# HJakeCunningham/ASVGP

Hardware: AMD Instinct MI355X
Metric: Mpoints/s per ELBO+grad step, N=10M 1D Matern-3/2 M=2048 (higher is better)
Workload: dtype f64

## Files before the change

### asvgp_amd/csrc/bcr_mfma.hpp

```cpp
#pragma once
#include "bcr.hpp"
#include "prior_plan.hpp"

namespace asvgp {

constexpr int BM_THREADS = 1024;
constexpr int BM_B = 4;
constexpr int BM_GAT = 0, BM_GBT = 16, BM_DINV = 32, BM_SD = 48, BM_CAT = 64, BM_CBT = 80, BM_W = 96, BM_DG = 100, BM_REC = 104;

__host__ __device__ inline size_t bcr_mfma_ws_doubles(long nb) { return (size_t)nb * BM_REC + 64; }
__host__ __device__ inline size_t bcr_mfma_lds_doubles(long nb) {
  return (size_t)((nb + 1) / 2 + 1) * 32 + (size_t)nb * 4 + 96 + (size_t)(BM_THREADS / 64) * 4 * 40 + (size_t)(nb / 8 + 2) * 52;
}

__device__ __forceinline__ double bm_mfma(double a, double b, double c) { return __builtin_amdgcn_mfma_f64_4x4x4f64(a, b, c, 0, 0, 0); }

__device__ __forceinline__ double bm_chol_linv(const double (&d)[10], int hi, int lo, double& dprod, int& badj) {
  double l00, i0, l10, l20, l30, l11, i1, l21, l31, l22, i2, l32, l33, i3;
  Num<double>::sqrt_inv(d[0], l00, i0);
  badj = !(d[0] > 0.0) ? 1 : 0;
  l10 = d[1] * i0; l20 = d[3] * i0; l30 = d[6] * i0;
  double s = fma(-l10, l10, d[2]);
  badj = (!(s > 0.0) && !badj) ? 2 : badj;
  Num<double>::sqrt_inv(s, l11, i1);
// ... 10 lines not shown
  const double z0 = (lo == 0) ? i0 : 0.0;
  const double z1 = fma(-l10, z0, (lo == 1) ? 1.0 : 0.0) * i1;
  const double z2 = fma(-l21, z1, fma(-l20, z0, (lo == 2) ? 1.0 : 0.0)) * i2;
  const double z3 = fma(-l32, z2, fma(-l31, z1, fma(-l30, z0, (lo == 3) ? 1.0 : 0.0))) * i3;
  return hi == 0 ? z0 : (hi == 1 ? z1 : (hi == 2 ? z2 : z3));
}

template <typename Src> __device__ __forceinline__ auto bm_src_load(const Src& A, int dd, long col, long M, int) -> decltype(A.load_dc(dd, col, M)) {
  return A.load_dc(dd, col, M);
}
template <typename Src> __device__ __forceinline__ double bm_src_load(const Src& A, int dd, long col, long M, long) {
  return A.load((long)dd * M + col, true);
}
struct BmLog {
  double m; int e;
  __device__ __forceinline__ void mul(double p) {
    m *= p;
    const int hi = __double2hiint(m);
    e += ((hi >> 20) & 0x7ff) - 1023;
    m = __hiloint2double((hi & 0x800fffff) | 0x3ff00000, __double2loint(m));
  }
};

__device__ __forceinline__ unsigned long long bm_wave_xor(unsigned long long x) {
#pragma unroll
  for (int off = 32; off > 0; off >>= 1) x ^= (unsigned long long)__shfl_xor((long long)x, off, 64);
  return x;
}
__device__ __forceinline__ void bm_msg_send(double* box, int n, double v, unsigned long long tag, int lane) {
  unsigned long long* b = reinterpret_cast<unsigned long long*>(box);
  const unsigned long long w = lane < n ? (unsigned long long)__double_as_longlong(v) : 0ull;
  const unsigned long long x = bm_wave_xor(w) ^ tag;
  if (lane < n) __hip_atomic_store(b + lane, w, __ATOMIC_RELAXED, __HIP_MEMORY_SCOPE_AGENT);
  if (lane == n) __hip_atomic_store(b + n, x, __ATOMIC_RELAXED, __HIP_MEMORY_SCOPE_AGENT);
}
__device__ __forceinline__ bool bm_msg_recv(const double* box, int n, double& v, unsigned long long tag, int lane, long spin_limit) {
  const unsigned long long* b = reinterpret_cast<const unsigned long long*>(box);
  for (long spins = 0; spins <= spin_limit; ++spins) {
    const unsigned long long w = lane <= n ? __hip_atomic_load(b + lane, __ATOMIC_RELAXED, __HIP_MEMORY_SCOPE_AGENT) : 0ull;
    const unsigned long long x = bm_wave_xor(lane < n ? w : 0ull) ^ tag;
    const unsigned long long chk = (unsigned long long)__shfl((long long)w, n, 64);
    if (x == chk) { v = __longlong_as_double((long long)w); return true; }
    __builtin_amdgcn_s_sleep(1);
  }
  return false;
}

struct BmSplit {
  int half = -1;
  double* xchg = nullptr;
  long spin_limit = 0;
  int* gave_up = nullptr;
  unsigned long long tag = 0;
};
constexpr int BM_XCHG = 96;

template <typename Src>
__device__ __attribute__((always_inline)) void bcr_mfma_solve(Src A, const double* rhs, int M, double* ws, double* lds, double* Sband, double* x,
                                                              double* logdet, int* info, int rhs_stride = 1, double* stamps = nullptr,
                                                              BmSplit sp = BmSplit{}) {
  constexpr int B = BM_B;
  const int tid = threadIdx.x;
  const int lane = tid & 63, wv = __builtin_amdgcn_readfirstlane(tid >> 6);
  const int r = lane >> 4, q = (lane >> 2) & 3, c = lane & 3;
  const int e = r * 4 + c, et = c * 4 + r;
  const int hi = r > c ? r : c, lo = r > c ? c : r;
  const int nb = (M + B - 1) / B;
  const int nslot = (nb + 1) / 2;
  double* Dl = lds;
  double* El = lds + (size_t)(nslot + 1) * 16;
  double* xs = El + (size_t)(nslot + 1) * 16;
  double* red = xs + (size_t)nb * B;
  double* slab = red + 96 + (size_t)(wv * 4 + q) * 40;
  double* Fl = red + 96 + (size_t)(BM_THREADS / 64) * 4 * 40;
  double* Sl = lds;
  int levels = 0;
  while ((1 << levels) < nb) ++levels;
  const bool split = sp.half >= 0;
  const int top = levels - 1, ht = 1 << (top > 0 ? top : 0);
  double s_other = 0.0;
  int bad_other = 0x7fffffff;
  auto level_share = [&](int l, int ne, int& m0, int& ne_h) {
    m0 = 0; ne_h = ne;
    if (!split) return;
    if (l < top) {
      const int mL = ht >> (l + 1);
      if (sp.half == 0) ne_h = ne < mL ? ne : mL;
      else { m0 = mL; ne_h = ne > mL ? ne - mL : 0; }
    } else {
      ne_h = sp.half == 0 ? ne : 0;
    }
  };
  int bad = 0;
  BmLog ld{1.0, 0};
  unsigned long long t_prev = stamps ? __builtin_amdgcn_s_memtime() : 0ull;
  int nst = 0;
  auto stamp = [&]() {
    if (stamps && tid == 0) { const unsigned long long t = __builtin_amdgcn_s_memtime(); stamps[nst++] = (double)(t - t_prev); t_prev = t; }
  };
  auto rec = [&](int node) -> double* { return ws + (size_t)node * BM_REC; };
  auto bandD = [&](int n, int rr, int cc) -> double {
    const int col = n * B + cc, row = n * B + rr;
    const bool pad = row >= M;
    const double v = bm_src_load(A, rr - cc, pad ? 0 : col, (long)M, 0);
    return pad ? ((rr == cc) ? 1.0 : 0.0) : v;
  };
// ... 264 lines not shown
        if (c == 0) xs[i * B + r] = w - gx;
        if (l >= 2) {
          double* Rw = Sl + (size_t)(i >> 2) * 48;
          Rw[e] = sii; Rw[16 + e] = -ncat; Rw[32 + e] = -ncbt;
        }
        if (l > 0) {
          double* Rw = rec(i);
          Rw[BM_SD + e] = sii; Rw[BM_CAT + e] = -ncat; Rw[BM_CBT + e] = -ncbt;
        }
        if (r >= c && i * B + r < M) Sband[(long)(r - c) * M + i * B + c] = sii;
        if (l == 0) {
          if (c <= r && i * B + c < M) Sband[(long)(B + c - r) * M + a * B + r] = -ncat;
          if (hasb && r <= c && b * B + r < M) Sband[(long)(B + r - c) * M + i * B + c] = -ncbt;
        }
      }
    }
    if (l == 1) __syncthreads(); else bcr_lds_barrier();
    if (split && l == top) {
      double* Rs = Sl + (size_t)(ht >> 2) * 48;
      if (sp.half == 0) {
        if (wv == 0) bm_msg_send(sp.xchg + 32, 52, lane < 48 ? Rs[lane < 48 ? lane : 0] : (lane < 52 ? xs[ht * B + lane - 48] : 0.0), sp.tag | 3ull, lane);
      } else {
        if (wv == 0) {
          double v = 0.0;
          if (!bm_msg_recv(sp.xchg + 32, 52, v, sp.tag | 3ull, lane, sp.spin_limit)) { if (lane == 0) *sp.gave_up = 1; }
          else if (lane < 48) {
            Rs[lane] = v;
            rec(ht)[BM_SD + lane] = v;
            if (lane < 16) {
              const int rr = lane >> 2, cc = lane & 3;
              if (rr >= cc && ht * B + rr < M) Sband[(long)(rr - cc) * M + ht * B + cc] = v;
            }
          } else if (lane < 52) {
            xs[ht * B + lane - 48] = v;
          }
        }
        __syncthreads();
        if (*sp.gave_up) return;
      }
    }
    stamp();
  }
  if (!(split && sp.half == 0))
    for (int col = M - B + tid; col < M; col += BM_THREADS)
      if (col >= 0)
#pragma unroll
        for (int dd = 1; dd <= B; ++dd)
          if (col + dd >= M) Sband[(long)dd * M + col] = 0.0;
  {
    const int row0 = (split && sp.half == 1) ? (ht + 1) * B : 0, row1 = (split && sp.half == 0) ? (ht + 1) * B : M;
    for (int row = row0 + tid; row < row1 && row < M; row += BM_THREADS) x[(long)row * rhs_stride] = xs[row];
  }
  if (!(split && sp.half == 1)) {
    const double mine = (r == 0 && c == 0) ? (log(ld.m) + (double)ld.e * 0.6931471805599453094) : 0.0;
    const double tot = wave_sum_dpp(mine);
    int bm = bad ? bad : 0x7fffffff;
#pragma unroll
    for (int off = 32; off > 0; off >>= 1) { const int o = __shfl_xor(bm, off, 64); bm = o < bm ? o : bm; }
    int* sbad = reinterpret_cast<int*>(red + 32);
    if (lane == 0) { red[wv] = tot; sbad[wv] = bm; }
    __syncthreads();
    if (split && tid == 0) { s_other = red[48]; bad_other = (int)red[49]; }
    if (tid == 0) {
      double s = 0.0;
      int bmin = 0x7fffffff;
      for (int w2 = 0; w2 < BM_THREADS / 64; ++w2) { s += red[w2]; bmin = sbad[w2] < bmin ? sbad[w2] : bmin; }
      s += s_other;
      bmin = bad_other < bmin ? bad_other : bmin;
      __hip_atomic_store(logdet + 0, 2.0 * s, __ATOMIC_RELAXED, __HIP_MEMORY_SCOPE_AGENT);
      __hip_atomic_store(logdet + 1, 0.0, __ATOMIC_RELAXED, __HIP_MEMORY_SCOPE_AGENT);
      __hip_atomic_store(info, (bmin == 0x7fffffff) ? 0 : bmin, __ATOMIC_RELAXED, __HIP_MEMORY_SCOPE_AGENT);
    }
  }
  stamp();
}


__host__ __device__ inline size_t bcr_mfma_pre_ws_doubles(long nb) { return (size_t)nb * 96 + 64; }
__host__ __device__ inline size_t bcr_mfma_pre_lds_doubles(long nb, int n_rec) {
  return PRIOR_TAB_HEADER + (size_t)2 * n_rec * prior_rec_fields(BM_B) + (size_t)(nb / 4 + 2) * 96 + (size_t)(nb + 1) / 2 + 64;
}

struct BmDual { double v, d; };
__device__ __forceinline__ BmDual bm_dmfma(BmDual x, BmDual y, BmDual c) {
  BmDual r;
  r.v = bm_mfma(x.v, y.v, c.v);
  r.d = bm_mfma(x.d, y.v, c.d);
  r.d = bm_mfma(x.v, y.d, r.d);
  return r;
}

__device__ __attribute__((always_inline)) void bcr_mfma_backward_pre(const double* __restrict__ tab, int n_rec, const int* __restrict__ node_rec, int M,
                                                                      double* ws, double* lds, double* Sv, double* Sd, double* logdet, int* info,
                                                                      unsigned long long* done_flag, unsigned long long seq,
                                                                      const unsigned long long* ready_flag = nullptr, long spin_limit = 0, int* gave_up = nullptr) {
  constexpr int B = BM_B, W = prior_rec_fields(B);
  const int tid = threadIdx.x;
  if (ready_flag) {
    if (tid == 0) {
      long spins = 0;
      while (__hip_atomic_load(ready_flag, __ATOMIC_RELAXED, __HIP_MEMORY_SCOPE_SYSTEM) < seq) {
        __builtin_amdgcn_s_sleep(8);
        if (++spins > spin_limit) { *gave_up = 1; break; }
      }
    }
    __syncthreads();
    if (*gave_up) return;
    __builtin_amdgcn_fence(__ATOMIC_ACQUIRE, "");
  }
// ... 107 lines not shown
```

### asvgp_amd/csrc/elbo.hip

```cpp
#include <stdlib.h>
#include <time.h>
#include <string.h>

#include "bcr_pre.hpp"
#include "bcr_mfma.hpp"
#include "handle.hpp"

namespace asvgp {


struct Ws {
  double *Kuu, *dK, *P, *LK, *dLK, *LP, *SK, *dSK, *SP, *c, *alpha, *logdets, *fin, *bcrK, *bcrP;
};
static size_t bcr_ws_chain(int planes, int k, bool big) {
  long ns = 1024;
  while ((long)planes * 2 * k * k * ns * 8 + 2 * ns * k * 8 + 1024 > 150 * 1024) ns >>= 1;
  if (big) ns *= 2;
  return (size_t)planes * (7 * k * k + k) * 2 * ns + (big ? (size_t)planes * k * k * ns : 0);
}
static size_t bcr_ws_K(int k, long M) {
  size_t a = bcr_ws_chain(2, k, false), b = bcr_ws_chain(2, k, true), c = bcr_pre_ws_doubles(k, (M + k - 1) / k);
  a = a > b ? a : b;
  return (a > c ? a : c) + 64;
}
// ... 348 lines not shown
    bcr_solve<double, K, 1, BandSumP, BIG>(BandSumP{A, Kuu, 1.0 / s}, b, M, wsP, lds, BandOut<double>{SP, nullptr}, x, logdets + 2, info + 1, nullptr, D);
    more_columns<K, BIG>(b, x, D, M, wsP, lds, lds_doubles);
  } else if (blockIdx.x == 1) {
    bcr_backward_pre<K>(tab, n_rec, node_rec, M, wsK, lds, BandOut<Dual>{SK, dSK}, logdets, info, done_flag, seq);
  } else {
    for (long e = (long)(blockIdx.x - 2) * blockDim.x + threadIdx.x; e < E; e += (long)fin.n_helpers * blockDim.x)
      assemble_band_slice(S_static, cf.c, cf.dc, cf.n, E, e, Kuu, dK);
    __syncthreads();
    if (threadIdx.x == 0) {
      __threadfence();
      __hip_atomic_fetch_add(fin.assembled, 1u, __ATOMIC_RELEASE, __HIP_MEMORY_SCOPE_AGENT);
    }
  }
  if (!fin.finalize) return;
  if (blockIdx.x < 2) {
    __syncthreads();
    if (threadIdx.x == 0) {
      __threadfence();
      __hip_atomic_fetch_add(fin.arrived, 1u, __ATOMIC_RELEASE, __HIP_MEMORY_SCOPE_AGENT);
    }
    return;
  }
  if (threadIdx.x == 0) {
    long spins = 0;
    while (__hip_atomic_load(fin.arrived, __ATOMIC_RELAXED, __HIP_MEMORY_SCOPE_AGENT) < 2u) {
      __builtin_amdgcn_s_sleep(8);
      if (++spins > (1L << 25)) { gave_up = 1; break; }
    }
  }
  __syncthreads();
  if (gave_up) { if (threadIdx.x == 0) atomicExch(info + 1, -1); return; }
  __builtin_amdgcn_fence(__ATOMIC_ACQUIRE, "agent");
  elbo_finalize_body<K>((int)blockIdx.x - 2, fin.n_helpers, lds, fin.stats, Kuu, dK, nullptr, nullptr, SK, dSK, SP, nullptr, x, logdets, (long)M, fin.D,
                        fin.th, fin.alpha_scale, fin.gacc, fin.ticket, fin.arrived, fin.out);
}

template <int K>
__global__ __launch_bounds__(BM_THREADS) void elbo_chains_mfma_kernel(KuuInterior ki, const double* S_static, KuuCoefs2 cf, double* Kuu, double* dK, const double* A, const double* b, int M,
                                                                      double* wsP, double* SP, double* x, double* logdets, int* info,
                                                                      double s, const double* tab, int n_rec, const int* node_rec,
                                                                      double* wsK, double* SK, double* dSK,
                                                                      unsigned long long* done_flag, unsigned long long seq,
                                                                      const unsigned long long* ready_flag, long spin_limit, FusedFin fin, const ThetaBox* box) {
  extern __shared__ double lds[];
  static_assert(K == BM_B, "matrix-core chains: bandwidth 4");
  const long E = (long)(K + 1) * M;
  const unsigned long long t_start = fin.debug_stamps ? __builtin_amdgcn_s_memrealtime() : 0ull;
  auto rstamp = [&](int slot) {
    if (fin.debug_stamps && threadIdx.x == 0 && blockIdx.x <= 2)
      logdets[(slot < 4 ? 8 + 4 * (int)blockIdx.x : 24) + slot] = (slot == 0) ? (double)(t_start & 0xffffffffull) : (double)((__builtin_amdgcn_s_memrealtime() - t_start) & 0xffffffffull);
  };
  rstamp(0);
  __shared__ int gave_up, kuu_ok;
  __shared__ double kuu_pref[4];
  if (threadIdx.x == 0) { gave_up = 0; kuu_ok = 0; }
  __syncthreads();
  double s_v = s, asc_v = fin.alpha_scale;
  ElboScalars th_v = fin.th;
  if (box) {
    if (threadIdx.x == 0) {
      long spins = 0;
      for (;;) {
        const unsigned long long got = __hip_atomic_load(&box->seq, __ATOMIC_RELAXED, __HIP_MEMORY_SCOPE_SYSTEM);
        if (got == seq) break;
        if (got == ~0ull || ++spins > spin_limit) { gave_up = 1; break; }
        __builtin_amdgcn_s_sleep(2);
      }
    }
    __syncthreads();
    if (gave_up) { if (threadIdx.x == 0) atomicExch(info + 1, -1); return; }
    s_v = box->s; asc_v = box->alpha_scale;
    th_v.v = box->v; th_v.l = box->l; th_v.s = box->s; th_v.N = box->N; th_v.Nw = box->Nw; th_v.cw = box->cw;
  }
  const double* stats = fin.stats;
  enum { LOGK, LOGP, TRKA, DTRKA, SKDK, SPDK, SKK, SPK, SPA, CC, AKA, ADKA, AAA, BA, NACC };
  double acc[NACC];
#pragma unroll
  for (int i = 0; i < NACC; ++i) acc[i] = 0.0;
  const bool isP = blockIdx.x == 0 || (fin.split && blockIdx.x == 2);
  const bool isPR = fin.split && blockIdx.x == 2;
  __shared__ double kdl[16];
  __shared__ double bnd[2 * PRIOR_BND_DIAGS * PRIOR_BND], dkb[2 * 5 * KI_DKB];
  {
    if (isP) rstamp(1);
    if (threadIdx.x == 0) {
      if (box) {
#pragma unroll
        for (int i = 0; i < 5; ++i) { kdl[i] = box->k[i]; kdl[8 + i] = box->dk[i]; }
      } else {
        kdl[0] = ki.k[0]; kdl[1] = ki.k[1]; kdl[2] = ki.k[2]; kdl[3] = ki.k[3]; kdl[4] = ki.k[4];
        kdl[8] = ki.dk[0]; kdl[9] = ki.dk[1]; kdl[10] = ki.dk[2]; kdl[11] = ki.dk[3]; kdl[12] = ki.dk[4];
      }
    }
    {
      const double* bnd_g = box ? box->bnd : reinterpret_cast<const double*>((const char*)__builtin_amdgcn_kernarg_segment_ptr() + offsetof(KuuInterior, bnd));
      const double* dkb_g = box ? box->dkb : reinterpret_cast<const double*>((const char*)__builtin_amdgcn_kernarg_segment_ptr() + offsetof(KuuInterior, dkb));
      if (threadIdx.x < 2 * PRIOR_BND_DIAGS * PRIOR_BND) bnd[threadIdx.x] = bnd_g[threadIdx.x];
      else if (threadIdx.x < 2 * PRIOR_BND_DIAGS * PRIOR_BND + 2 * 5 * KI_DKB) dkb[threadIdx.x - 2 * PRIOR_BND_DIAGS * PRIOR_BND] = dkb_g[threadIdx.x - 2 * PRIOR_BND_DIAGS * PRIOR_BND];
    }
    __syncthreads();
  }
  if (isP) {
    BmSplit bsp;
    if (fin.split) { bsp.half = isPR ? 1 : 0; bsp.xchg = fin.xchg; bsp.spin_limit = spin_limit; bsp.gave_up = &gave_up; bsp.tag = seq << 8; }
    bcr_mfma_solve<BandSumToep>(BandSumToep{A, 1.0 / s_v, (lds_cdouble_ptr)kdl, (lds_cdouble_ptr)bnd, ki.lo, ki.hi}, b, M, wsP, lds, SP, x, logdets + 2, info + 1, 1,
                                fin.debug_stamps ? (isPR ? fin.xchg + 128 : logdets + 32) : (double*)nullptr, bsp);
    rstamp(3);
    __syncthreads();
    if (gave_up) { if (threadIdx.x == 0) atomicExch(info + 1, -1); return; }
    rstamp(4);
    if (fin.finalize) {
      const double* xs_l = lds + (size_t)2 * ((((M + K - 1) / K) + 1) / 2 + 1) * 16;
      static_assert(BM_THREADS == 1024, "two columns per thread");
      int nbl = (M + K - 1) / K, lv = 0;
      while ((1 << lv) < nbl) ++lv;
      const long jsep = (long)(1 << (lv > 0 ? lv - 1 : 0)) * K;
      const long j0 = isPR ? jsep : 0, j1 = (fin.split && !isPR) ? jsep : (long)M;
      unsigned long long kw = 0ull;
      const bool kuu_reader = !isPR && (threadIdx.x >> 6) == 1;
      if (kuu_reader && (threadIdx.x & 63) <= 4)
        kw = __hip_atomic_load(reinterpret_cast<const unsigned long long*>(fin.gacc + 8) + (threadIdx.x & 63), __ATOMIC_RELAXED, __HIP_MEMORY_SCOPE_AGENT);
      double sp[2][K + 1], av[2][K + 1], bj[2];
#pragma unroll
      for (int cI = 0; cI < 2; ++cI) {
        const long j = j0 + threadIdx.x + cI * BM_THREADS, jc = j < j1 ? j : j1 - 1;
#pragma unroll
        for (int r = 0; r <= K; ++r) { sp[cI][r] = SP[(long)r * M + jc]; av[cI][r] = stats[(long)r * M + jc]; }
        bj[cI] = stats[(long)(K + 1) * M + jc];
      }
#pragma unroll
      for (int cI = 0; cI < 2; ++cI) {
        const long j = j0 + threadIdx.x + cI * BM_THREADS;
        if (j >= j1) continue;
        const bool left = j < ki.lo, right = j >= ki.hi;
        const double xj = xs_l[j];
#pragma unroll
        for (int r = 0; r <= K; ++r) {
          const long o = (long)r * M + j;
          const double w2 = (r == 0) ? 1.0 : 2.0;
          double kv = kdl[r], dkv = kdl[8 + r];
          if (left || right) {
            kv = bnd[left ? (long)r * PRIOR_BND + j : (long)(PRIOR_BND_DIAGS + r) * PRIOR_BND + (j - ki.hi)];
            if (ki.dk_tab) {
              dkv = dkb[left ? (long)r * KI_DKB + j : (long)(5 + r) * KI_DKB + (j - ki.hi)];
            } else {
              dkv = 0.0;
              for (int t = 0; t < cf.n; ++t) dkv = fma(box ? box->dc[t] : cf.dc[t], S_static[(long)t * E + o], dkv);
            }
          }
          const double xx = (j + r < M) ? w2 * xj * xs_l[j + r] : 0.0;
          acc[SPDK] = fma(w2 * sp[cI][r], dkv, acc[SPDK]);
          acc[SPK] = fma(w2 * sp[cI][r], kv, acc[SPK]);
          acc[SPA] = fma(w2 * sp[cI][r], av[cI][r], acc[SPA]);
          acc[AKA] = fma(kv, xx, acc[AKA]);
          acc[ADKA] = fma(dkv, xx, acc[ADKA]);
          acc[AAA] = fma(av[cI][r], xx, acc[AAA]);
        }
        acc[BA] = fma(bj[cI], xj, acc[BA]);
      }
      if (kuu_reader) {
        const int ln = threadIdx.x & 63;
        const unsigned long long x = bm_wave_xor(ln < 4 ? kw : 0ull) ^ ((seq << 8) | 4ull);
        const unsigned long long chk = (unsigned long long)__shfl((long long)kw, 4, 64);
        if (x == chk) { if (ln < 4) kuu_pref[ln] = __longlong_as_double((long long)kw); if (ln == 0) kuu_ok = 1; }
      }
    }
  } else {
    if (fin.debug_no_assembly) {
      if (threadIdx.x == 0) { for (long sp_ = 0; sp_ < spin_limit; ++sp_) __builtin_amdgcn_s_sleep(8); atomicExch(info + 1, -1); }
      return;
    }
    bcr_mfma_backward_pre(tab, n_rec, node_rec, M, wsK, lds, SK, dSK, logdets, info, done_flag, seq, ready_flag,
                          spin_limit < (1L << 20) ? spin_limit : (1L << 20), &gave_up);
    if (gave_up) { if (threadIdx.x == 0) atomicExch(info + 1, -1); return; }
    rstamp(1);
    if (fin.finalize) {
      __syncthreads();
      double sk[2][K + 1], dsk[2][K + 1], av[2][K + 1];
#pragma unroll
      for (int cI = 0; cI < 2; ++cI) {
        const long j = (long)threadIdx.x + cI * BM_THREADS, jc = j < M ? j : M - 1;
#pragma unroll
        for (int r = 0; r <= K; ++r) { sk[cI][r] = SK[(long)r * M + jc]; dsk[cI][r] = dSK[(long)r * M + jc]; av[cI][r] = stats[(long)r * M + jc]; }
      }
#pragma unroll
      for (int cI = 0; cI < 2; ++cI) {
        const long j = (long)threadIdx.x + cI * BM_THREADS;
        if (j >= M) continue;
        const bool left = j < ki.lo, right = j >= ki.hi;
#pragma unroll
        for (int r = 0; r <= K; ++r) {
          const long o = (long)r * M + j;
          const double w2 = (r == 0) ? 1.0 : 2.0;
          double kv = kdl[r], dkv = kdl[8 + r];
          if (left || right) {
            kv = bnd[left ? (long)r * PRIOR_BND + j : (long)(PRIOR_BND_DIAGS + r) * PRIOR_BND + (j - ki.hi)];
            if (ki.dk_tab) {
              dkv = dkb[left ? (long)r * KI_DKB + j : (long)(5 + r) * KI_DKB + (j - ki.hi)];
            } else {
              dkv = 0.0;
              for (int t = 0; t < cf.n; ++t) dkv = fma(box ? box->dc[t] : cf.dc[t], S_static[(long)t * E + o], dkv);
            }
          }
          acc[TRKA] = fma(w2 * sk[cI][r], av[cI][r], acc[TRKA]);
          acc[DTRKA] = fma(w2 * dsk[cI][r], av[cI][r], acc[DTRKA]);
          acc[SKDK] = fma(w2 * sk[cI][r], dkv, acc[SKDK]);
          acc[SKK] = fma(w2 * sk[cI][r], kv, acc[SKK]);
        }
      }
    }
  }
  if (!fin.finalize) { rstamp(2); return; }
  if (isP) rstamp(5);
  double* part0 = lds;
  const int lane = threadIdx.x & 63;
  double mine[8];
  mine[0] = isP ? acc[SPDK] : acc[TRKA];
  mine[1] = isP ? acc[SPK] : acc[DTRKA];
  mine[2] = isP ? acc[SPA] : acc[SKDK];
  mine[3] = isP ? acc[AKA] : acc[SKK];
  mine[4] = acc[ADKA]; mine[5] = acc[AAA]; mine[6] = acc[BA]; mine[7] = 0.0;
  const int nmine = isP ? 7 : 4;
  __syncthreads();
  const bool b0 = (lane & 1) != 0, b1 = (lane & 2) != 0, b2 = (lane & 4) != 0;
  double s4[4], s2[2];
#pragma unroll
  for (int i = 0; i < 4; ++i) { const double keep = b0 ? mine[4 + i] : mine[i], send = b0 ? mine[i] : mine[4 + i]; s4[i] = keep + dpp_move_f64<0xB1>(send); }
#pragma unroll
  for (int i = 0; i < 2; ++i) { const double keep = b1 ? s4[2 + i] : s4[i], send = b1 ? s4[i] : s4[2 + i]; s2[i] = keep + dpp_move_f64<0x4E>(send); }
  double s1 = (b2 ? s2[1] : s2[0]) + dpp_xor4_f64(b2 ? s2[0] : s2[1], b2);
  s1 += dpp_move_f64<0x128>(s1); s1 += __shfl_xor(s1, 16, 64); s1 += __shfl_xor(s1, 32, 64);
  const int wv = threadIdx.x >> 6;
  if (lane < 8) part0[wv * 8 + lane] = s1;
  __syncthreads();
  if (threadIdx.x >= 64) return;
  double t2 = part0[(2 * (lane >> 3)) * 8 + (lane & 7)] + part0[(2 * (lane >> 3) + 1) * 8 + (lane & 7)];
  t2 += __shfl_xor(t2, 8, 64); t2 += __shfl_xor(t2, 16, 64); t2 += __shfl_xor(t2, 32, 64);
  double red[7];
  red[0] = __shfl(t2, 0, 64); red[1] = __shfl(t2, 4, 64); red[2] = __shfl(t2, 2, 64); red[3] = __shfl(t2, 6, 64);
  red[4] = __shfl(t2, 1, 64); red[5] = __shfl(t2, 5, 64); red[6] = __shfl(t2, 3, 64);
  (void)nmine;
  double tot[NACC];
#pragma unroll
  for (int i = 0; i < NACC; ++i) tot[i] = 0.0;
  if (isP && threadIdx.x == 0) rstamp(6);
  const unsigned long long mtag = seq << 8;
  double* box_kuu = fin.gacc + 8;
  double* box_pr = fin.gacc + FIN_GACC_PR;
  if (!isP || isPR) {
    double v = red[0];
#pragma unroll
    for (int i = 1; i < 7; ++i) v = (lane == i) ? red[i] : v;
    bm_msg_send(isPR ? box_pr : box_kuu, nmine, v, mtag | (isPR ? 5ull : 4ull), lane);
    if (threadIdx.x == 0) rstamp(2);
    return;
  }
  double kuu_v = 0.0, pr_v = 0.0;
  {
    bool ok = true;
    if (kuu_ok) kuu_v = lane < 4 ? kuu_pref[lane] : 0.0;
    else ok = bm_msg_recv(box_kuu, 4, kuu_v, mtag | 4ull, lane, spin_limit);
    if (ok && fin.split) ok = bm_msg_recv(box_pr, 7, pr_v, mtag | 5ull, lane, spin_limit);
    if (!ok) { if (lane == 0) atomicExch(info + 1, -1); return; }
  }
  {
    const int pidx[7] = {SPDK, SPK, SPA, AKA, ADKA, AAA, BA};
#pragma unroll
    for (int i = 0; i < 7; ++i) tot[pidx[i]] = red[i] + (fin.split ? __shfl(pr_v, i, 64) : 0.0);
  }
  tot[TRKA] = __shfl(kuu_v, 0, 64); tot[DTRKA] = __shfl(kuu_v, 1, 64); tot[SKDK] = __shfl(kuu_v, 2, 64); tot[SKK] = __shfl(kuu_v, 3, 64);
  if (threadIdx.x != 0) return;
#pragma unroll
  for (int i = 0; i < 14; ++i) __hip_atomic_store(fin.gacc + i, 0.0, __ATOMIC_RELAXED, __HIP_MEMORY_SCOPE_AGENT);
  {
    const double v = th_v.v, sn = th_v.s, N = th_v.N, Nw = th_v.Nw;
    const double yy = stats[(long)(K + 1) * M + M];
    const double asc = asc_v;
    tot[AKA] *= asc * asc; tot[ADKA] *= asc * asc; tot[AAA] *= asc * asc; tot[BA] *= asc;
    tot[LOGK] = __hip_atomic_load(logdets + 0, __ATOMIC_RELAXED, __HIP_MEMORY_SCOPE_AGENT);
    tot[LOGP] = __hip_atomic_load(logdets + 2, __ATOMIC_RELAXED, __HIP_MEMORY_SCOPE_AGENT);
    tot[CC] = tot[BA] / sn;
    const double two_pi = 6.283185307179586476925286766559;
    double elbo = -0.5 * N * log(two_pi * sn);
    elbo -= 0.5 * tot[LOGP];
    elbo += 0.5 * tot[LOGK];
    elbo -= 0.5 * yy / sn;
    elbo += 0.5 * tot[CC];
    elbo -= 0.5 * Nw * v / sn;
    elbo += 0.5 * tot[TRKA] / sn;
    if (th_v.cw != 0.0) elbo += th_v.cw;
    const double d_l = 0.5 * (tot[SKDK] - tot[SPDK] - tot[ADKA] + tot[DTRKA] / sn);
    const double d_v = 0.5 * (-tot[SKK] / v + tot[SPK] / v + tot[AKA] / v + tot[TRKA] / (v * sn)) - 0.5 * Nw / sn;
    const double s2 = sn * sn;
    const double d_s = -0.5 * N / sn + 0.5 * tot[SPA] / s2 + 0.5 * yy / s2 + 0.5 * tot[AAA] / s2 - tot[BA] / s2 + 0.5 * Nw * v / s2 - 0.5 * tot[TRKA] / s2;
    double* out = fin.out;
    out[0] = elbo; out[1] = d_v; out[2] = d_l; out[3] = d_s;
    out[4] = tot[LOGK]; out[5] = tot[LOGP]; out[6] = tot[TRKA]; out[7] = tot[CC];
    if (fin.mirror) {
      double* m = fin.mirror;
      const double mv[10] = {elbo, d_v, d_l, d_s, tot[LOGK], tot[LOGP], tot[TRKA], tot[CC],
                             (double)__hip_atomic_load(info, __ATOMIC_RELAXED, __HIP_MEMORY_SCOPE_AGENT),
                             (double)__hip_atomic_load(info + 1, __ATOMIC_RELAXED, __HIP_MEMORY_SCOPE_AGENT)};
      double sum = (double)fin.mirror_seq;
#pragma unroll
      for (int i = 0; i < 10; ++i) { __hip_atomic_store(m + i, mv[i], __ATOMIC_RELAXED, __HIP_MEMORY_SCOPE_SYSTEM); sum += mv[i]; }
      __hip_atomic_store(m + 11, sum, __ATOMIC_RELAXED, __HIP_MEMORY_SCOPE_SYSTEM);
      __hip_atomic_store(m + 10, (double)fin.mirror_seq, __ATOMIC_RELAXED, __HIP_MEMORY_SCOPE_SYSTEM);
    }
  }
  rstamp(2);
}

static __global__ void scale_sub_kernel(const double* __restrict__ a, const double* __restrict__ b, double* __restrict__ o,
                                 long n) {
  long i = (long)blockIdx.x * blockDim.x + threadIdx.x;
  if (i < n) o[i] = a[i] - b[i];
}
static __global__ void scale_kernel(double* __restrict__ x, double f, long n) {
  long i = (long)blockIdx.x * blockDim.x + threadIdx.x;
  if (i < n) x[i] = x[i] * f;
}

template <int K, bool TANGENT>
static int run_chains(Handle* h, const double* stats, const double* S, int kind, double v, double l, double s, long M, long D,
                      Ws w, int* info, hipStream_t st, bool& use_bcr, int part = 0, bool scale_alpha = true, FusedFin* fin = nullptr) {
  double t_enter = 0.0;
  if (debug_env().host_times) { timespec ts; clock_gettime(CLOCK_MONOTONIC, &ts); t_enter = ts.tv_sec * 1e6 + ts.tv_nsec * 1e-3; }
  KuuCoefs2 cf;
  for (int t = 0; t < ASVGP_MAX_KUU_TERMS; ++t) cf.c[t] = cf.dc[t] = 0.0;
  int rc = asvgp_matern_coeffs(kind, v, l, cf.c, cf.dc, &cf.n);
  if (rc) return rc;
  const long E = (long)(K + 1) * M;
  const double* A = stats;
  const double* b = stats ? stats + E : nullptr;
  const long nb = (M + K - 1) / K;
  const int algo = h->band_algo;
  const bool have_plan = h->plan && prior_plan_M(h->plan) == M && prior_plan_k(h->plan) == K && prior_plan_terms(h->plan) == cf.n;
  if ((algo == 3 || algo == 4) && !have_plan) { set_error("band algorithms 3 and 4 need asvgp_prior_plan_1d for this (M, k, kernel)"); return ASVGP_ERR_BAD_ARG; }
  size_t ldsK = sizeof(double) * (TANGENT ? bcr_lds_doubles<Dual, K, 0>(nb) : bcr_lds_doubles<double, K, 0>(nb));
  size_t ldsP = sizeof(double) * bcr_lds_doubles<double, K, 1>(nb);
  bool planned = have_plan && (algo == 0 || algo == 3 || algo == 4);
  size_t lds_bytes = planned ? ldsP : (ldsK > ldsP ? ldsK : ldsP);
  bool fits = lds_bytes <= 160 * 1024 - 256;
  bool big = false;
  constexpr bool HAS_BIG = (K <= 5);
  if (HAS_BIG && !fits) {
    size_t bK = sizeof(double) * (TANGENT ? bcr_lds_doubles<Dual, K, 0, true>(nb) : bcr_lds_doubles<double, K, 0, true>(nb));
    size_t bP = sizeof(double) * bcr_lds_doubles<double, K, 1, true>(nb);
    size_t bb = planned ? bP : (bK > bP ? bK : bP);
    if (bb <= 160 * 1024 - 256) { big = true; fits = true; lds_bytes = bb; }
  }
  use_bcr = (algo == 2 || algo == 3 || algo == 4 || (algo == 0 && fits));
  planned = planned && use_bcr;
  if (part != 0 && (!use_bcr || planned)) {
    if (part == 1) return ASVGP_OK;
    part = 0;
  }
  if (planned) {
    const int n_rec = prior_plan_nrec(h->plan);
    bool use_mfma = false;
    KuuInterior ki;
// ... 657 lines not shown
```

### asvgp_amd/csrc/phi_pass.hip

```cpp
#include <stdlib.h>

#include "handle.hpp"

namespace asvgp {

constexpr int PHI_THREADS = 1024;
constexpr int PHI_CH = 32;
constexpr int PHI_MAX_BLOCKS = 256;
constexpr size_t PHI_LDS_BUDGET = 160 * 1024 - 512;

template <int K> struct FxTab {
  int g[K + 1];
  constexpr FxTab() : g{} {
    double cf[K + 1][K + 1] = {};
    for (int i = 0; i <= K; ++i)
      for (int p = 0; p <= K; ++p) cf[i][p] = piece_coef<K, 0>(i, p);
    for (int d = 0; d <= K; ++d) {
      double mx = 0.0;
      for (int i = 0; i + d <= K; ++i)
        for (int q = 0; q <= 32; ++q) {
          const double t = q / 32.0;
          double a = cf[i][K], b = cf[i + d][K];
          for (int p = K - 1; p >= 0; --p) { a = a * t + cf[i][p]; b = b * t + cf[i + d][p]; }
          if (a * b > mx) mx = a * b;
// ... 646 lines not shown
  if (r >= nrows_probe) return;
  const long base = ((long)r * row_stride) & ~1L;
  if (base + 128 > N) return;
  const double xa = x[base + 2 * lane], xb = x[base + 2 * lane + 1];
  const int ca = mq_guess(xa, m0, inv_delta, n_mesh), cb = mq_guess(xb, m0, inv_delta, n_mesh);
  const int c0 = __builtin_amdgcn_readfirstlane(ca);
  bool good = true;
  if (!__all(ca == c0 && cb == c0)) {
    const unsigned long long d0 = __ballot(ca != c0), d1 = __ballot(cb != c0);
    const int c1 = d0 ? __builtin_amdgcn_readlane(ca, (int)__builtin_ctzll(d0)) : __builtin_amdgcn_readlane(cb, (int)__builtin_ctzll(d1 | (1ull << 63)));
    good = __all((ca - c0 <= 2 && c0 - ca <= 2) || (ca - c1 <= 2 && c1 - ca <= 2)) && __all((cb - c0 <= 2 && c0 - cb <= 2) || (cb - c1 <= 2 && c1 - cb <= 2));
  }
  if (lane == 0 && good) atomicAdd(count, 1);
}

static bool handle_phi_is_series(Handle* h, const double* x, long N, double m0, double inv_delta, long n_mesh, hipStream_t st) {
  if (h->phi_order == 1) return false;
  if (h->phi_order == 2) return true;
  for (int i = 0; i < h->n_order_seen; ++i)
    if (h->order_seen[i].ptr == x && h->order_seen[i].n == N) return h->order_seen[i].series != 0;
  int series = 0;
  const int nprobe = 512;
  if (N >= 128L * nprobe) {
    if (!h->order_dev && hipMalloc(&h->order_dev, sizeof(int)) != hipSuccess) h->order_dev = nullptr;
    int cnt = 0;
    if (h->order_dev && hipMemsetAsync(h->order_dev, 0, sizeof(int), st) == hipSuccess) {
      hipLaunchKernelGGL(phi_order_probe_kernel, dim3(nprobe), dim3(64), 0, st, x, N, N / nprobe, nprobe, m0, inv_delta, (int)n_mesh, h->order_dev);
      if (hipMemcpyAsync(&cnt, h->order_dev, sizeof(int), hipMemcpyDeviceToHost, st) == hipSuccess && hipStreamSynchronize(st) == hipSuccess)
        series = cnt * 10 >= nprobe * 9 ? 1 : 0;
    }
  }
  if (h->n_order_seen < 8) h->order_seen[h->n_order_seen++] = Handle::OrderSeen{x, N, series};
  return series != 0;
}

template <int K, int TP, int TS>
static int launch_phi_sort_as(Handle* h, const double* x, const double* y, long N, const double* mesh, long n_mesh, double delta,
                              long M, double* stats, double* ws, hipStream_t st, double step, double m0, double m_last, double margin) {
  size_t lds_bytes = ps_lds_bytes<K, TP, TS>();
  if (ps_epilogue_bytes<K>() > lds_bytes) lds_bytes = ps_epilogue_bytes<K>();
  if (lds_bytes > 160 * 1024) return 1;
  long nblk = (N + TP * PS_THREADS - 1) / (TP * PS_THREADS);
  const long gmax = (h->phi_blocks > 0 && h->phi_blocks < PHI_MAX_BLOCKS) ? h->phi_blocks : PHI_MAX_BLOCKS;
  const int G = (int)(nblk < 1 ? 1 : (nblk > gmax ? gmax : nblk));
  long ppb = (N + G - 1) / G;
  ppb = TS ? ((ppb + 127) & ~127L) : ((ppb + 1) & ~1L);
  if (ppb > 0x3fffffffL) return 1;
  PsArgs a;
  a.x = x; a.y = y; a.N = N; a.mesh_g = mesh; a.n_mesh = (int)n_mesh; a.inv_delta = 1.0 / delta; a.M = (int)M;
  a.m0 = m0; a.m_last = m_last; a.step = step; a.smax_fast = 0.5 - margin;
  a.partials = ws; a.ppb = ppb; a.zero_ptr = stats; a.zero_n = (K + 2) * M + 1; a.stamps = nullptr; a.stamps_wave = 0;
  a.ranges = reinterpret_cast<int*>(ws + (size_t)PHI_MAX_BLOCKS * ((size_t)(K + 2) * M + 1));
  auto kern = phi_sort_kernel<K, TP, 0, 1, TS>;
  hipError_t e = hipFuncSetAttribute(reinterpret_cast<const void*>(kern), hipFuncAttributeMaxDynamicSharedMemorySize, (int)lds_bytes);
  if (e != hipSuccess) { set_error("hipFuncSetAttribute(%zu B LDS): %s", lds_bytes, hipGetErrorString(e)); return ASVGP_ERR_LDS_CAPACITY; }
  const bool prof = h->prof_on && h->prof_n < PROF_RING && (h->prof_calls++ % h->prof_every == 0);
  if (prof) (void)hipEventRecord(h->prof_ev[h->prof_n][0], st);
  hipLaunchKernelGGL(kern, dim3((unsigned)G), dim3(PS_THREADS), lds_bytes, st, a);
  if (prof) { (void)hipEventRecord(h->prof_ev[h->prof_n][1], st); ++h->prof_n; }
  h->phi_last_series = TS;
  const int E1 = (int)((K + 2) * M + 1);
  const int gsplit = G >= 64 ? 16 : (G >= 8 ? 4 : 1);
  if (h->phi_defer) {
    h->pend = Handle::PendingReduce{a.partials, G, (int)M, K, stats, true, a.ranges};
    return check_launch("phi_accumulate_1d (tile sort, reduce deferred)");
  }
  hipLaunchKernelGGL(phi_reduce_kernel, dim3((E1 + 255) / 256, gsplit), dim3(256), 0, st, a.partials, G, (int)M, K, 0, M, 1L, 0, 1, stats, (const int*)a.ranges);
  return check_launch("phi_accumulate_1d (tile sort)");
}

template <int K>
static int launch_phi_sort(Handle* h, const double* x, const double* y, long N, long D, const double* mesh, long n_mesh, double delta,
                           long M, double* stats, double* ws, hipStream_t st) {
  if (D != 1 || N < 2 || M > PS_NCELL || ((reinterpret_cast<uintptr_t>(x) | reinterpret_cast<uintptr_t>(y)) & 15) != 0) return 1;
  double step = 0.0, m0 = 0.0, m_last = 0.0;
  if (!handle_mesh_is_linspace(h, mesh, n_mesh, st, &step, &m0, &m_last)) return 1;
  const double amax = fabs(m0) > fabs(m_last) ? fabs(m0) : fabs(m_last);
  const double margin = 16.0 * 2.220446049250313e-16 * amax / delta + 1e-12;
  if (!(margin < 0.125)) return 1;
  constexpr int TP = ps_tile_points<K>();
  constexpr int TPS = TP < 4 ? TP : 4;
  if (handle_phi_is_series(h, x, N, m0, 1.0 / delta, n_mesh, st)) {
    const int rc = launch_phi_sort_as<K, TPS, 1>(h, x, y, N, mesh, n_mesh, delta, M, stats, ws, st, step, m0, m_last, margin);
    if (rc != 1) return rc;
  }
  return launch_phi_sort_as<K, TP, 0>(h, x, y, N, mesh, n_mesh, delta, M, stats, ws, st, step, m0, m_last, margin);
}

template <int K>
static int launch_phi(Handle* h, const double* x, const double* y, long N, long D, const double* mesh, long n_mesh,
                      double delta, long M, double* stats, double* partials, hipStream_t st) {
  { const int rcf = handle_flush_phi_reduce(h, nullptr, st); if (rcf) return rcf; }
  const int ncells = (int)n_mesh - 1;
  if (h->phi_algo == 0 || h->phi_algo == 6) {
    const int rc = launch_phi_sort<K>(h, x, y, N, D, mesh, n_mesh, delta, M, stats, partials, st);
    if (rc != 1) { h->phi_last = 6; return rc; }
    if (h->phi_algo == 6) { set_error("phi algorithm 6 (tile sort) needs D == 1, N >= 2, M <= 2048, 16-byte aligned x / y and a mesh that is an exact linspace"); return ASVGP_ERR_UNSUPPORTED; }
  }
  if (h->phi_algo == 0 || h->phi_algo == 5) {
    const int rc = launch_phi_moments<K>(h, x, y, N, D, mesh, n_mesh, delta, M, stats, partials, st);
    if (rc != 1) { h->phi_last = 5; return rc; }
    if (h->phi_algo == 5) { set_error("phi algorithm 5 (centred moments) needs D == 1, 16-byte aligned x / y and M small enough for the LDS split"); return ASVGP_ERR_UNSUPPORTED; }
  }
  const bool fx = (h->phi_algo != 1);
  h->phi_last = fx ? 3 : 1;
  int maxc = phi_max_cols(K, n_mesh, fx);
  if (maxc < 2 * K + 2) {
    set_error("phi_accumulate_1d: mesh table (%ld knots) leaves no LDS for the band", n_mesh);
// ... 284 lines not shown
```

Baseline: 136,100.

## Fold log-determinant and info reductions into fused finalize message path

The P-chain solve now hands its per-lane log-determinant and failure code back to the caller instead of doing its own block reduction and global atomic stores. Those values ride along in the existing finalize reduction and cross-block messages, and the Kuu logdet and info travel in two extra message slots. This removes global atomic reloads of logdets and info in the finisher. It also precomputes reciprocals so divides become multiplies, and caches the hipFuncSetAttribute call in the phi launcher to cut host overhead. The risk is subtle correctness issues: the static granted cache is keyed only by device, not by kernel template instance, and the message protocol layout has changed.

```diff
diff --git a/asvgp_amd/csrc/bcr_mfma.hpp b/asvgp_amd/csrc/bcr_mfma.hpp
--- a/asvgp_amd/csrc/bcr_mfma.hpp
+++ b/asvgp_amd/csrc/bcr_mfma.hpp
@@ -86,6 +86,8 @@
   long spin_limit = 0;
   int* gave_up = nullptr;
   unsigned long long tag = 0;
+  double* ld_lane = nullptr;
+  int* bad_lane = nullptr;
 };
 constexpr int BM_XCHG = 96;
 
@@ -456,9 +458,20 @@
     for (int row = row0 + tid; row < row1 && row < M; row += BM_THREADS) x[(long)row * rhs_stride] = xs[row];
   }
   if (!(split && sp.half == 1)) {
-    const double mine = (r == 0 && c == 0) ? (log(ld.m) + (double)ld.e * 0.6931471805599453094) : 0.0;
+    double mine = (r == 0 && c == 0) ? (log(ld.m) + (double)ld.e * 0.6931471805599453094) : 0.0;
+    int bm = bad ? bad : 0x7fffffff;
+    if (sp.ld_lane) {
+      if (split && tid == 0) {
+        mine += red[48];
+        const int bo = (int)red[49];
+        bm = bo < bm ? bo : bm;
+      }
+      *sp.ld_lane = mine;
+      *sp.bad_lane = bm;
+      stamp();
+      return;
+    }
     const double tot = wave_sum_dpp(mine);
-    int bm = bad ? bad : 0x7fffffff;
 #pragma unroll
     for (int off = 32; off > 0; off >>= 1) { const int o = __shfl_xor(bm, off, 64); bm = o < bm ? o : bm; }
     int* sbad = reinterpret_cast<int*>(red + 32);
diff --git a/asvgp_amd/csrc/elbo.hip b/asvgp_amd/csrc/elbo.hip
--- a/asvgp_amd/csrc/elbo.hip
+++ b/asvgp_amd/csrc/elbo.hip
@@ -424,7 +424,7 @@
   };
   rstamp(0);
   __shared__ int gave_up, kuu_ok;
-  __shared__ double kuu_pref[4];
+  __shared__ double kuu_pref[6];
   if (threadIdx.x == 0) { gave_up = 0; kuu_ok = 0; }
   __syncthreads();
   double s_v = s, asc_v = fin.alpha_scale;
@@ -472,9 +472,12 @@
     }
     __syncthreads();
   }
+  double ld_part = 0.0, kuu_ld = 0.0, kuu_info = 0.0, yy_pre = 0.0;
+  int bad_part = 0x7fffffff;
   if (isP) {
     BmSplit bsp;
     if (fin.split) { bsp.half = isPR ? 1 : 0; bsp.xchg = fin.xchg; bsp.spin_limit = spin_limit; bsp.gave_up = &gave_up; bsp.tag = seq << 8; }
+    if (fin.finalize) { bsp.ld_lane = &ld_part; bsp.bad_lane = &bad_part; }
     bcr_mfma_solve<BandSumToep>(BandSumToep{A, 1.0 / s_v, (lds_cdouble_ptr)kdl, (lds_cdouble_ptr)bnd, ki.lo, ki.hi}, b, M, wsP, lds, SP, x, logdets + 2, info + 1, 1,
                                 fin.debug_stamps ? (isPR ? fin.xchg + 128 : logdets + 32) : (double*)nullptr, bsp);
     rstamp(3);
@@ -490,7 +493,7 @@
       const long j0 = isPR ? jsep : 0, j1 = (fin.split && !isPR) ? jsep : (long)M;
       unsigned long long kw = 0ull;
       const bool kuu_reader = !isPR && (threadIdx.x >> 6) == 1;
-      if (kuu_reader && (threadIdx.x & 63) <= 4)
+      if (kuu_reader && (threadIdx.x & 63) <= 6)
         kw = __hip_atomic_load(reinterpret_cast<const unsigned long long*>(fin.gacc + 8) + (threadIdx.x & 63), __ATOMIC_RELAXED, __HIP_MEMORY_SCOPE_AGENT);
       double sp[2][K + 1], av[2][K + 1], bj[2];
 #pragma unroll
@@ -500,6 +503,7 @@
         for (int r = 0; r <= K; ++r) { sp[cI][r] = SP[(long)r * M + jc]; av[cI][r] = stats[(long)r * M + jc]; }
         bj[cI] = stats[(long)(K + 1) * M + jc];
       }
+      if (!isPR) yy_pre = stats[(long)(K + 1) * M + M];
 #pragma unroll
       for (int cI = 0; cI < 2; ++cI) {
         const long j = j0 + threadIdx.x + cI * BM_THREADS;
@@ -532,9 +536,9 @@
       }
       if (kuu_reader) {
         const int ln = threadIdx.x & 63;
-        const unsigned long long x = bm_wave_xor(ln < 4 ? kw : 0ull) ^ ((seq << 8) | 4ull);
-        const unsigned long long chk = (unsigned long long)__shfl((long long)kw, 4, 64);
-        if (x == chk) { if (ln < 4) kuu_pref[ln] = __longlong_as_double((long long)kw); if (ln == 0) kuu_ok = 1; }
+        const unsigned long long x = bm_wave_xor(ln < 6 ? kw : 0ull) ^ ((seq << 8) | 4ull);
+        const unsigned long long chk = (unsigned long long)__shfl((long long)kw, 6, 64);
+        if (x == chk) { if (ln < 6) kuu_pref[ln] = __longlong_as_double((long long)kw); if (ln == 0) kuu_ok = 1; }
       }
     }
   } else {
@@ -546,6 +550,7 @@
                           spin_limit < (1L << 20) ? spin_limit : (1L << 20), &gave_up);
     if (gave_up) { if (threadIdx.x == 0) atomicExch(info + 1, -1); return; }
     rstamp(1);
+    kuu_ld = lds[0]; kuu_info = lds[2];
     if (fin.finalize) {
       __syncthreads();
       double sk[2][K + 1], dsk[2][K + 1], av[2][K + 1];
@@ -591,8 +596,10 @@
   mine[1] = isP ? acc[SPK] : acc[DTRKA];
   mine[2] = isP ? acc[SPA] : acc[SKDK];
   mine[3] = isP ? acc[AKA] : acc[SKK];
-  mine[4] = acc[ADKA]; mine[5] = acc[AAA]; mine[6] = acc[BA]; mine[7] = 0.0;
-  const int nmine = isP ? 7 : 4;
+  mine[4] = acc[ADKA]; mine[5] = acc[AAA]; mine[6] = acc[BA];
+  const bool finisher = isP && !isPR;
+  mine[7] = finisher ? ld_part : 0.0;
+  const int nmine = isP ? 7 : 6;
   __syncthreads();
   const bool b0 = (lane & 1) != 0, b1 = (lane & 2) != 0, b2 = (lane & 4) != 0;
   double s4[4], s2[2];
@@ -604,6 +611,13 @@
   s1 += dpp_move_f64<0x128>(s1); s1 += __shfl_xor(s1, 16, 64); s1 += __shfl_xor(s1, 32, 64);
   const int wv = threadIdx.x >> 6;
   if (lane < 8) part0[wv * 8 + lane] = s1;
+  int* bad0 = reinterpret_cast<int*>(part0 + (BM_THREADS / 64) * 8);
+  if (finisher) {
+    int bmn = bad_part;
+#pragma unroll
+    for (int off = 32; off > 0; off >>= 1) { const int o = __shfl_xor(bmn, off, 64); bmn = o < bmn ? o : bmn; }
+    if (lane == 0) bad0[wv] = bmn;
+  }
   __syncthreads();
   if (threadIdx.x >= 64) return;
   double t2 = part0[(2 * (lane >> 3)) * 8 + (lane & 7)] + part0[(2 * (lane >> 3) + 1) * 8 + (lane & 7)];
@@ -611,7 +625,7 @@
   double red[7];
   red[0] = __shfl(t2, 0, 64); red[1] = __shfl(t2, 4, 64); red[2] = __shfl(t2, 2, 64); red[3] = __shfl(t2, 6, 64);
   red[4] = __shfl(t2, 1, 64); red[5] = __shfl(t2, 5, 64); red[6] = __shfl(t2, 3, 64);
-  (void)nmine;
+  const double ld_sum = __shfl(t2, 7, 64);
   double tot[NACC];
 #pragma unroll
   for (int i = 0; i < NACC; ++i) tot[i] = 0.0;
@@ -623,15 +637,27 @@
     double v = red[0];
 #pragma unroll
     for (int i = 1; i < 7; ++i) v = (lane == i) ? red[i] : v;
+    if (!isP) v = (lane == 4) ? kuu_ld : ((lane == 5) ? kuu_info : v);
     bm_msg_send(isPR ? box_pr : box_kuu, nmine, v, mtag | (isPR ? 5ull : 4ull), lane);
     if (threadIdx.x == 0) rstamp(2);
     return;
   }
+  const double v = th_v.v, sn = th_v.s, N = th_v.N, Nw = th_v.Nw;
+  const double den = lane == 0 ? sn : (lane == 1 ? v : (lane == 2 ? sn * sn : v * sn));
+  const double rcp = 1.0 / den;
+  const double inv_s = __shfl(rcp, 0, 64), inv_v = __shfl(rcp, 1, 64), inv_s2 = __shfl(rcp, 2, 64), inv_vs = __shfl(rcp, 3, 64);
+  const double two_pi = 6.283185307179586476925286766559;
+  const double lg = log(two_pi * sn);
+  int bmin = lane < BM_THREADS / 64 ? bad0[lane] : 0x7fffffff;
+#pragma unroll
+  for (int off = 8; off > 0; off >>= 1) { const int o = __shfl_xor(bmin, off, 64); bmin = o < bmin ? o : bmin; }
+  bmin = __shfl(bmin, 0, 64);
+  const int info_p = (bmin == 0x7fffffff) ? 0 : bmin;
   double kuu_v = 0.0, pr_v = 0.0;
   {
     bool ok = true;
-    if (kuu_ok) kuu_v = lane < 4 ? kuu_pref[lane] : 0.0;
-    else ok = bm_msg_recv(box_kuu, 4, kuu_v, mtag | 4ull, lane, spin_limit);
+    if (kuu_ok) kuu_v = lane < 6 ? kuu_pref[lane] : 0.0;
+    else ok = bm_msg_recv(box_kuu, 6, kuu_v, mtag | 4ull, lane, spin_limit);
     if (ok && fin.split) ok = bm_msg_recv(box_pr, 7, pr_v, mtag | 5ull, lane, spin_limit);
     if (!ok) { if (lane == 0) atomicExch(info + 1, -1); return; }
   }
@@ -641,44 +667,44 @@
     for (int i = 0; i < 7; ++i) tot[pidx[i]] = red[i] + (fin.split ? __shfl(pr_v, i, 64) : 0.0);
   }
   tot[TRKA] = __shfl(kuu_v, 0, 64); tot[DTRKA] = __shfl(kuu_v, 1, 64); tot[SKDK] = __shfl(kuu_v, 2, 64); tot[SKK] = __shfl(kuu_v, 3, 64);
+  tot[LOGK] = __shfl(kuu_v, 4, 64);
+  const double info_k = (double)(int)__shfl(kuu_v, 5, 64);
   if (threadIdx.x != 0) return;
-#pragma unroll
-  for (int i = 0; i < 14; ++i) __hip_atomic_store(fin.gacc + i, 0.0, __ATOMIC_RELAXED, __HIP_MEMORY_SCOPE_AGENT);
   {
-    const double v = th_v.v, sn = th_v.s, N = th_v.N, Nw = th_v.Nw;
-    const double yy = stats[(long)(K + 1) * M + M];
+    const double yy = yy_pre;
     const double asc = asc_v;
     tot[AKA] *= asc * asc; tot[ADKA] *= asc * asc; tot[AAA] *= asc * asc; tot[BA] *= asc;
-    tot[LOGK] = __hip_atomic_load(logdets + 0, __ATOMIC_RELAXED, __HIP_MEMORY_SCOPE_AGENT);
-    tot[LOGP] = __hip_atomic_load(logdets + 2, __ATOMIC_RELAXED, __HIP_MEMORY_SCOPE_AGENT);
-    tot[CC] = tot[BA] / sn;
-    const double two_pi = 6.283185307179586476925286766559;
-    double elbo = -0.5 * N * log(two_pi * sn);
+    tot[LOGP] = 2.0 * ld_sum;
+    tot[CC] = tot[BA] * inv_s;
+    double elbo = -0.5 * N * lg;
     elbo -= 0.5 * tot[LOGP];
     elbo += 0.5 * tot[LOGK];
-    elbo -= 0.5 * yy / sn;
+    elbo -= 0.5 * yy * inv_s;
     elbo += 0.5 * tot[CC];
-    elbo -= 0.5 * Nw * v / sn;
-    elbo += 0.5 * tot[TRKA] / sn;
+    elbo -= 0.5 * Nw * v * inv_s;
+    elbo += 0.5 * tot[TRKA] * inv_s;
     if (th_v.cw != 0.0) elbo += th_v.cw;
-    const double d_l = 0.5 * (tot[SKDK] - tot[SPDK] - tot[ADKA] + tot[DTRKA] / sn);
-    const double d_v = 0.5 * (-tot[SKK] / v + tot[SPK] / v + tot[AKA] / v + tot[TRKA] / (v * sn)) - 0.5 * Nw / sn;
-    const double s2 = sn * sn;
-    const double d_s = -0.5 * N / sn + 0.5 * tot[SPA] / s2 + 0.5 * yy / s2 + 0.5 * tot[AAA] / s2 - tot[BA] / s2 + 0.5 * Nw * v / s2 - 0.5 * tot[TRKA] / s2;
-    double* out = fin.out;
-    out[0] = elbo; out[1] = d_v; out[2] = d_l; out[3] = d_s;
-    out[4] = tot[LOGK]; out[5] = tot[LOGP]; out[6] = tot[TRKA]; out[7] = tot[CC];
+    const double d_l = 0.5 * (tot[SKDK] - tot[SPDK] - tot[ADKA] + tot[DTRKA] * inv_s);
+    const double d_v = 0.5 * (-tot[SKK] * inv_v + tot[SPK] * inv_v + tot[AKA] * inv_v + tot[TRKA] * inv_vs) - 0.5 * Nw * inv_s;
+    const double d_s = -0.5 * N * inv_s + 0.5 * tot[SPA] * inv_s2 + 0.5 * yy * inv_s2 + 0.5 * tot[AAA] * inv_s2 - tot[BA] * inv_s2 + 0.5 * Nw * v * inv_s2 -
+                       0.5 * tot[TRKA] * inv_s2;
+    const double mv[10] = {elbo, d_v, d_l, d_s, tot[LOGK], tot[LOGP], tot[TRKA], tot[CC], info_k, (double)info_p};
     if (fin.mirror) {
       double* m = fin.mirror;
-      const double mv[10] = {elbo, d_v, d_l, d_s, tot[LOGK], tot[LOGP], tot[TRKA], tot[CC],
-                             (double)__hip_atomic_load(info, __ATOMIC_RELAXED, __HIP_MEMORY_SCOPE_AGENT),
-                             (double)__hip_atomic_load(info + 1, __ATOMIC_RELAXED, __HIP_MEMORY_SCOPE_AGENT)};
       double sum = (double)fin.mirror_seq;
 #pragma unroll
       for (int i = 0; i < 10; ++i) { __hip_atomic_store(m + i, mv[i], __ATOMIC_RELAXED, __HIP_MEMORY_SCOPE_SYSTEM); sum += mv[i]; }
       __hip_atomic_store(m + 11, sum, __ATOMIC_RELAXED, __HIP_MEMORY_SCOPE_SYSTEM);
       __hip_atomic_store(m + 10, (double)fin.mirror_seq, __ATOMIC_RELAXED, __HIP_MEMORY_SCOPE_SYSTEM);
     }
+    double* out = fin.out;
+#pragma unroll
+    for (int i = 0; i < 8; ++i) out[i] = mv[i];
+    __hip_atomic_store(logdets + 2, tot[LOGP], __ATOMIC_RELAXED, __HIP_MEMORY_SCOPE_AGENT);
+    __hip_atomic_store(logdets + 3, 0.0, __ATOMIC_RELAXED, __HIP_MEMORY_SCOPE_AGENT);
+    __hip_atomic_store(info + 1, info_p, __ATOMIC_RELAXED, __HIP_MEMORY_SCOPE_AGENT);
+#pragma unroll
+    for (int i = 0; i < 15; ++i) __hip_atomic_store(fin.gacc + i, 0.0, __ATOMIC_RELAXED, __HIP_MEMORY_SCOPE_AGENT);
   }
   rstamp(2);
 }
diff --git a/asvgp_amd/csrc/phi_pass.hip b/asvgp_amd/csrc/phi_pass.hip
--- a/asvgp_amd/csrc/phi_pass.hip
+++ b/asvgp_amd/csrc/phi_pass.hip
@@ -722,8 +722,13 @@
   a.partials = ws; a.ppb = ppb; a.zero_ptr = stats; a.zero_n = (K + 2) * M + 1; a.stamps = nullptr; a.stamps_wave = 0;
   a.ranges = reinterpret_cast<int*>(ws + (size_t)PHI_MAX_BLOCKS * ((size_t)(K + 2) * M + 1));
   auto kern = phi_sort_kernel<K, TP, 0, 1, TS>;
-  hipError_t e = hipFuncSetAttribute(reinterpret_cast<const void*>(kern), hipFuncAttributeMaxDynamicSharedMemorySize, (int)lds_bytes);
-  if (e != hipSuccess) { set_error("hipFuncSetAttribute(%zu B LDS): %s", lds_bytes, hipGetErrorString(e)); return ASVGP_ERR_LDS_CAPACITY; }
+  static size_t lds_granted[16] = {0};
+  size_t& granted = lds_granted[h->device & 15];
+  if (lds_bytes > granted) {
+    hipError_t e = hipFuncSetAttribute(reinterpret_cast<const void*>(kern), hipFuncAttributeMaxDynamicSharedMemorySize, (int)lds_bytes);
+    if (e != hipSuccess) { set_error("hipFuncSetAttribute(%zu B LDS): %s", lds_bytes, hipGetErrorString(e)); return ASVGP_ERR_LDS_CAPACITY; }
+    granted = lds_bytes;
+  }
   const bool prof = h->prof_on && h->prof_n < PROF_RING && (h->prof_calls++ % h->prof_every == 0);
   if (prof) (void)hipEventRecord(h->prof_ev[h->prof_n][0], st);
   hipLaunchKernelGGL(kern, dim3((unsigned)G), dim3(PS_THREADS), lds_bytes, st, a);
```

After: 136,600 (median of 6 runs). Within noise of the previous version (+0.4%).
